# tkoolen/Parametron.jl

Hardware: AMD Instinct MI355X
Metric: QP re-evaluations/sec (Q,q,C,d rebuild) at n=4096 (higher is better)
Workload: dtype f64; 1 GPU; C2 dense least-squares QP: n=4096 vars, A 4096x4096, m=512 equality rows, fp64; canonical Q,q,const + C,d MOI triplets; n=4096, r=4096, m=512, objective_mode=canonical, instances_per_gpu=1, parallelism=single GPU, replay=tape

## Files before the change

parametron.jl_amd/csrc/gram.hip:

```cpp
#include <algorithm>
#include <memory>
#include <vector>

#include "streams.h"

#ifndef PMT_GRAM_ABL_NO_LINEAR
#define PMT_GRAM_ABL_NO_LINEAR 0
#endif

namespace pmt {

constexpr size_t PAIR_FLAG_BYTES = 4096;
constexpr int DELIVER_ORDER_W = 1;

__global__ __launch_bounds__(256) void gram_linear_kernel(const double *__restrict__ A, int64_t lda, int64_t rows, int64_t cols,
                                                          const int64_t *__restrict__ xvar, const double *__restrict__ b, int sign,
                                                          int moi, const int64_t *__restrict__ varmap, LT *__restrict__ out_lin) {
    const int64_t col = (int64_t)blockIdx.x * 4 + (threadIdx.x >> 6);
    if (col >= cols) return;
    const int lane = threadIdx.x & 63;
    const double *a = A + col * lda;
    double acc = 0.0;
    if (b && sign)
        for (int64_t i = lane; i < rows; i += 64) acc += signed_const(b[i], sign) * a[i];
// ... 218 lines not shown
static int release_group(const DeliverPlan &d, SideStream *side, int grp, hipStream_t s) {
    const dma::Signal flag{0, reinterpret_cast<int64_t *>(static_cast<char *>(side->counters) + FLAGS_OFFSET) + grp};
    return dma::launch_signal_store(d.sig->engine ? d.sig->dep[grp] : flag, s);
}

static int deliver_submit(const DeliverPlan &d, SideStream *side) {
    if (!d.sig->engine) {
        char *cb = static_cast<char *>(side->counters);
        if (int rc = launch_courier(d.src, d.host_dev, reinterpret_cast<long long *>(cb + FLAGS_OFFSET), reinterpret_cast<unsigned *>(cb + DONE_OFFSET),
                                    side->err_dev, d.ngroups, d.gbeg, d.gend, side->fetch)) return rc;
        PMT_HIP_CHECK(hipEventRecord(side->fetch_done, side->fetch));
        side->fetch_pending = true;
        return PMT_OK;
    }
    auto submit = [p = d]() -> int {
        for (int i = 0; i < p.ngroups; ++i)
            if (int rc = dma::copy_to_host(p.sig->eng, p.host + p.gbeg[i], p.src + p.gbeg[i], sizeof(double) * (size_t)(p.gend[i] - p.gbeg[i]),
                                           &p.sig->dep[i], p.sig->done, 1)) return rc;
        return PMT_OK;
    };
    d.sig->pending = true;
    side->dma_pending.emplace_back(d.sig->eng, d.sig->done);
    side->keepalive.push_back(d.sig);
    if (!side->in_replay) return submit();
    side->deferred.push_back(submit);
    return PMT_OK;
}

static int fork_side(SideStream *side, hipStream_t s) {
    PMT_HIP_CHECK(hipEventRecord(side->fork, s));
    PMT_HIP_CHECK(hipStreamWaitEvent(side->stream, side->fork, 0));
    return PMT_OK;
}

static int fused_node(const GramArgs &g, SideStream *side, hipStream_t s) {
    int rc = launch_gram_tall(g.A, g.lda, g.rows, g.cols, g.xvar, g.b, g.sign, g.moi, g.varmap, g.out_quad, g.out_csc, g.alpha, g.out_lin,
                              g.out_const, g.workspace, s);
    if (!rc && side && side->in_replay) rc = fork_side(side, s);
    const int64_t nt = cdiv(g.cols, ST);
    if (!rc && nt > 1)
        rc = launch_gram_sk(g.A, g.lda, g.rows, g.cols, g.xvar, g.varmap, g.moi, g.out_quad, g.out_csc, g.alpha, g.workspace, 0, 0, nt * (nt - 1) / 2,
                            nullptr, 0, nullptr, s, 1);
    return rc;
}

static int mid_node(const GramArgs &g, SideStream *side, hipStream_t s) {
    PMT_REQUIRE(side && side->counters && (size_t)gram_mid_counters(g.cols) * sizeof(unsigned) <= MID_COUNTER_BYTES, PMT_STATE_ERROR,
                "quad_gram: no auxiliary state for this stream");
    int rc = launch_gram_mid(g.A, g.lda, g.rows, g.cols, g.xvar, g.b, g.sign, g.moi, g.varmap, g.out_quad, g.out_csc, g.alpha, g.out_lin,
                             g.out_const, g.workspace, reinterpret_cast<unsigned *>(static_cast<char *>(side->counters) + MID_OFFSET), s);
    return !rc && side->in_replay ? fork_side(side, s) : rc;
}

static int stream_k_node(const GramArgs &g, bool staged, const DeliverPlan &d, SideStream *side, hipStream_t s) {
    hipStream_t s2 = side ? side->stream : s;
    if (side) { if (int rc = fork_side(side, s)) return rc; }
    const int64_t rows = g.rows, cols = g.cols;
    int rc = PMT_OK;
    double *scratch = g.workspace ? reinterpret_cast<double *>(static_cast<char *>(g.workspace) + gram_sk_workspace_bytes(rows, cols)) : nullptr;
    const int nsplit = (scratch && g.b && g.sign) ? linear_splits(rows, cols) : 1;
    if (PMT_GRAM_ABL_NO_LINEAR) {
    } else if (cols > 0 && nsplit > 1) {
        const int64_t chunk = 64 * cdiv(cdiv(rows, nsplit), 64);
        PMT_LAUNCH(gram_linear_split_kernel, dim3((unsigned)cdiv(cols, 4), (unsigned)nsplit), dim3(256), 0, s2, g.A, g.lda, rows, cols, g.b, g.sign, chunk, scratch);
        PMT_LAUNCH(gram_linear_finish_kernel, dim3((unsigned)cdiv(cols, 256)), dim3(256), 0, s2, scratch, nsplit, cols, g.xvar, g.moi, g.varmap, g.out_lin);
        rc = check_launch("gram_linear_split_kernel");
    } else if (cols > 0) {
        PMT_LAUNCH(gram_linear_kernel, dim3((unsigned)cdiv(cols, 4)), dim3(256), 0, s2, g.A, g.lda, rows, cols, g.xvar, g.b, g.sign, g.moi, g.varmap, g.out_lin);
        rc = check_launch("gram_linear_kernel");
    }
    double *chains = scratch ? scratch + (size_t)linear_splits(rows, cols) * (size_t)cols : nullptr;
    const int order = constant_order(staged ? GramForm::StreamKStaged : GramForm::StreamK, rows, cols).order;
    auto const_part = [=]() -> int {
        int rc2 = PMT_OK;
        if (order == 5) rc2 = launch_gram_mid_constant(g.b, g.sign, rows, g.out_const, s2);
        else if (g.b && g.sign && rows > 0) rc2 = launch_blocked_dot(g.b, g.sign, g.b, g.sign, rows, chains, g.out_const, s2, order);
        else if (hipMemsetAsync(g.out_const, 0, sizeof(double), s2) != hipSuccess) rc2 = fail(PMT_HIP_ERROR, "hipMemsetAsync(out_const)");
        if (side) { PMT_HIP_CHECK(hipEventRecord(side->join2, side->stream)); PMT_HIP_CHECK(hipStreamWaitEvent(s, side->join2, 0)); }
        return rc2;
    };
    const bool defer_const = side && side->in_replay;
    if (!rc && defer_const) side->deferred.push_back(const_part);
    if (side) PMT_HIP_CHECK(hipEventRecord(side->join, side->stream));
    if (!rc && cols > 0 && !staged) rc = launch_gram_sk(g.A, g.lda, rows, cols, g.xvar, g.varmap, g.moi, g.out_quad, g.out_csc, g.alpha, g.workspace, 0, 0, -1,
                                                        nullptr, 0, nullptr, s);
    else if (!rc && cols > 0) {
        unsigned *pair_flags = g.workspace ? reinterpret_cast<unsigned *>(static_cast<char *>(g.workspace) + gram_sk_workspace_bytes(rows, cols) - PAIR_FLAG_BYTES) : nullptr;
        if (pair_flags) PMT_HIP_CHECK(hipMemsetAsync(pair_flags, 0, PAIR_FLAG_BYTES, s));
        for (int st = 0; !rc && st < d.nstages; ++st) {
// ... 103 lines not shown
```

parametron.jl_amd/csrc/gram_mid.hip:

```cpp
#include "gram_common.h"

#ifndef PMT_MID_WPS
#define PMT_MID_WPS 1
#endif
#ifndef PMT_MID_G
#define PMT_MID_G 256
#endif
#ifndef PMT_MID_MAXWG
#define PMT_MID_MAXWG 2304
#endif
#ifndef PMT_MID_D
#define PMT_MID_D 2
#endif
#ifndef PMT_MID_GROUP_US
#define PMT_MID_GROUP_US 1.15
#endif
#ifndef PMT_MID_TAIL_US
#define PMT_MID_TAIL_US 0.95
#endif
#ifndef PMT_MID_SB
#define PMT_MID_SB 8
#endif
#ifndef PMT_MID_FB
#define PMT_MID_FB 4
#endif
#ifndef PMT_MID_FORMAL
#if defined(__HIP_DEVICE_COMPILE__) && !defined(__gfx950__) && !defined(__gfx942__)
#define PMT_MID_FORMAL 1
#else
#define PMT_MID_FORMAL 0
#endif
#endif

#ifdef PMT_MID_TRACE
__device__ unsigned long long g_mid_trace[1024 * 8];
#define MID_STAMP(k) do { if (threadIdx.x == 0 && blockIdx.x < 1024) g_mid_trace[blockIdx.x * 8 + (k)] = wall_clock64(); } while (0)
extern "C" int pmt_mid_trace_read(unsigned long long *host) {
    return hipMemcpyFromSymbol(host, HIP_SYMBOL(g_mid_trace), sizeof(unsigned long long) * 1024 * 8) == hipSuccess ? 0 : 1;
}
#else
#define MID_STAMP(k) do { } while (0)
#endif

namespace pmt {

constexpr int MT = 64;
constexpr int MACC = 64;
constexpr int MPART = MACC * 64;
constexpr int MSTRIDE = MPART + MT + 8;
constexpr int MPITCH = MT + 1;
constexpr int MFG = 8;
constexpr int MCNT = 16;
constexpr int MQBUF = 4 * 2048;
constexpr int MFLAG = MQBUF + 4 * MT;
constexpr int MMAPS = MFLAG + 8;
constexpr int MSH = MMAPS + 2 * MT;

struct MidArgs {
    const double *A; int64_t lda, rows, cols;
    const double *b; int sign;
    const int64_t *xvar; const int64_t *varmap; int moi;
    QT *out_quad; double *out_csc; double alpha; LT *out_lin; double *out_const;
    int nb;
    int n_off, s_off, s_diag;
    int gpc_off, gpc_diag;
    int n_tail, s_tail, gpc_tail;
    double *ws;
    unsigned *counters;
    int xcd;
    int persist, total;
    unsigned *tickets;
};

struct MidPlan { int nb, n_off, s_off, s_diag, gpc_off, gpc_diag, n_tail, s_tail, gpc_tail, wgs; };
// ... 128 lines not shown
        for (int tm = 0; tm < (DIAG ? c + 1 : 4); ++tm) {
            const int a = (tm * 4 + c) * 4;
            acc[a] = __builtin_amdgcn_mfma_f64_4x4x4f64(buf[tm].y, bv[c][0].y, acc[a], 0, 0, 0);
        }
    __builtin_amdgcn_sched_barrier(0);
#pragma unroll
    for (int c = 0; c < NC; ++c) {
#pragma unroll
        for (int r = 1; r < 4; ++r)
#pragma unroll
            for (int tm = 0; tm < (DIAG ? c + 1 : 4); ++tm) {
                const int a = (tm * 4 + c) * 4 + r;
                acc[a] = __builtin_amdgcn_mfma_f64_4x4x4f64(buf[tm].x, bv[c][r].x, acc[a], 0, 0, 0);
            }
#pragma unroll
        for (int r = 1; r < 4; ++r)
#pragma unroll
            for (int tm = 0; tm < (DIAG ? c + 1 : 4); ++tm) {
                const int a = (tm * 4 + c) * 4 + r;
                acc[a] = __builtin_amdgcn_mfma_f64_4x4x4f64(buf[tm].y, bv[c][r].y, acc[a], 0, 0, 0);
            }
    }
    if (DIAG) {
        const double c0 = signed_const(cb.x, sign), c1 = signed_const(cb.y, sign);
#pragma unroll
        for (int t = 0; t < 4; ++t) qacc[t] = __builtin_amdgcn_mfma_f64_4x4x4f64(buf[t].x, c0, qacc[t], 0, 0, 0);
#pragma unroll
        for (int t = 0; t < 4; ++t) qacc[t] = __builtin_amdgcn_mfma_f64_4x4x4f64(buf[t].y, c1, qacc[t], 0, 0, 0);
    }
}

#define MID_SB() __builtin_amdgcn_sched_barrier(0)
template <bool DIAG>
__device__ __forceinline__ void mid_step(const MidArgs &g, double *__restrict__ rot, int64_t next_row0, unsigned (&voff)[DIAG ? 4 : 8],
                                         f64x2 (&buf)[DIAG ? 4 : 8], f64x2 &cb, int sign, int lane, double (&acc)[MACC], double (&qacc)[4]) {
    constexpr int BO = DIAG ? 0 : 4;
    const int lm = lane & 15, lrow = lane & 48, lk = lane >> 4;
    const char *base = reinterpret_cast<const char *>(g.A + next_row0);
    auto reload = [&](int t) {
        asm volatile("" : "+v"(voff[t]));
        buf[t] = *reinterpret_cast<const f64x2 *>(base + voff[t]);
    };
    f64x2 bv[4][4];
#pragma unroll
    for (int c = 0; c < 4; ++c) bv[c][0] = buf[BO + c];
    auto lds_op = [&](int i) {
        if (i < 4) *reinterpret_cast<f64x2 *>(rot + (i * 64 + lane) * 2) = buf[BO + i];
        else {
            const int c = (i - 4) / 3, r = 1 + (i - 4) % 3;
            bv[c][r] = *reinterpret_cast<const f64x2 *>(rot + (c * 64 + lrow + ((lm + 4 * r) & 15)) * 2);
        }
    };
    MID_SB();
    int k = 0;
#pragma unroll
    for (int pass = 0; pass < 2; ++pass)
#pragma unroll
        for (int c = 0; c < 4; ++c)
#pragma unroll
            for (int tm = 0; tm < (DIAG ? c + 1 : 4); ++tm) {
                const int a = (tm * 4 + c) * 4;
                acc[a] = __builtin_amdgcn_mfma_f64_4x4x4f64(pass ? buf[tm].y : buf[tm].x, pass ? bv[c][0].y : bv[c][0].x, acc[a], 0, 0, 0);
                if (k < 16) { MID_SB(); lds_op(k); MID_SB(); }
                ++k;
            }
    if (DIAG) {
        const double c0 = signed_const(cb.x, sign), c1 = signed_const(cb.y, sign);
#pragma unroll
        for (int t = 0; t < 4; ++t) qacc[t] = __builtin_amdgcn_mfma_f64_4x4x4f64(buf[t].x, c0, qacc[t], 0, 0, 0);
#pragma unroll
        for (int t = 0; t < 4; ++t) qacc[t] = __builtin_amdgcn_mfma_f64_4x4x4f64(buf[t].y, c1, qacc[t], 0, 0, 0);
        MID_SB();
        cb = *reinterpret_cast<const f64x2 *>((g.b ? g.b : g.A) + next_row0 + 2 * lk);
    }
// ... 182 lines not shown
#endif
}

template <bool DIAG>
__device__ __forceinline__ void mid_fold(const double *p, int count, int64_t stride, int tid, double (&sum)[16], double &qs) {
#pragma unroll
    for (int u = 0; u < 16; ++u) sum[u] = 0.0;
    qs = 0.0;
    for (int c0 = 0; c0 < count; c0 += PMT_MID_FB) {
        double v[PMT_MID_FB][16], qv[PMT_MID_FB];
#pragma unroll
        for (int cc = 0; cc < PMT_MID_FB; ++cc) {
            const double *pc = p + (int64_t)min(c0 + cc, count - 1) * stride;
#pragma unroll
            for (int u = 0; u < 16; ++u) {
                const int a = (tid >> 6) + 4 * u;
                v[cc][u] = 0.0;
                if (mid_used(DIAG, a)) v[cc][u] = mid_get(pc + tid + 256 * u);
            }
            qv[cc] = 0.0;
            if (DIAG && tid < MT) qv[cc] = mid_get(pc + MPART + tid);
        }
#pragma unroll
        for (int cc = 0; cc < PMT_MID_FB; ++cc) {
            const bool live = c0 + cc < count;
#pragma unroll
            for (int u = 0; u < 16; ++u) { const double t = sum[u] + v[cc][u]; sum[u] = live ? t : sum[u]; }
            const double t = qs + qv[cc];
            qs = live ? t : qs;
        }
    }
}

template <bool DIAG, bool FAST>
__device__ __forceinline__ void mid_body(const MidArgs &g, double *sh, int tid, int jb, int kb, int chunk, int nchunk, int gpc, int first_wg, unsigned *counter) {
    constexpr int NG = DIAG ? 4 : 8;
    constexpr int D = PMT_MID_D;
    const int lane = tid & 63;
    const int wave = __builtin_amdgcn_readfirstlane(tid >> 6);
    const int lm = lane & 15, lk = lane >> 4;
    const int64_t cj0 = (int64_t)jb * MT, ck0 = (int64_t)kb * MT;
    const int ngroups = (int)((g.rows + 7) >> 3);
    const int g0 = chunk * gpc + wave, g1 = min((chunk + 1) * gpc, ngroups);
    const int my = g1 > g0 ? (g1 - g0 + 3) / 4 : 0;
    const bool ragged = FAST && (g.rows & 7) && my > 0 && g0 + 4 * (my - 1) == ngroups - 1;
    const int nfast = ragged ? my - 1 : my;

    MID_STAMP(0);
    mid_maps(g, sh, tid, jb, kb);
    double acc[MACC], qacc[4] = {0.0, 0.0, 0.0, 0.0};
#pragma unroll
    for (int a = 0; a < MACC; ++a) acc[a] = 0.0;
    unsigned voff[NG];
#pragma unroll
    for (int t = 0; t < NG; ++t) voff[t] = (unsigned)((min((t < 4 ? cj0 : ck0) + 16 * (t & 3) + lm, g.cols - 1) * g.lda + 2 * lk) * 8);
    double *rot = sh + wave * 512;
    f64x2 buf[D][NG], cb[D];
    auto row_of = [&](int s) { return (int64_t)(g0 + 4 * min(s, max(nfast - 1, 0))) * 8; };
    if (nfast > 0) {
#pragma unroll
        for (int d = 0; d < D; ++d) mid_load<DIAG, FAST>(g, row_of(d), lane, cj0, ck0, voff, buf[d], cb[d]);
        if (FAST) {
            int s0 = 0;
            for (; s0 + D <= nfast; s0 += D) {
#pragma unroll
                for (int d = 0; d < D; ++d) mid_step<DIAG>(g, rot, row_of(s0 + d + D), voff, buf[d], cb[d], g.sign, lane, acc, qacc);
            }
#pragma unroll
            for (int d = 0; d < D - 1; ++d)
                if (s0 + d < nfast) mid_compute<DIAG>(rot, buf[d], cb[d], g.sign, lane, acc, qacc);
        } else {
            for (int s0 = 0; s0 < nfast; s0 += D) {
#pragma unroll
                for (int d = 0; d < D; ++d) {
                    if (s0 + d < nfast) mid_compute<DIAG>(rot, buf[d], cb[d], g.sign, lane, acc, qacc);
                    mid_load<DIAG, FAST>(g, row_of(s0 + d + D), lane, cj0, ck0, voff, buf[d], cb[d]);
                }
            }
        }
    }
    if (ragged) {
        mid_load<DIAG, false>(g, (int64_t)(ngroups - 1) * 8, lane, cj0, ck0, voff, buf[0], cb[0]);
        mid_compute<DIAG>(rot, buf[0], cb[0], g.sign, lane, acc, qacc);
    }

    MID_STAMP(1);
    unsigned *flag = reinterpret_cast<unsigned *>(sh + MFLAG);
    double *w = g.ws + (int64_t)(first_wg + chunk) * MSTRIDE;
    __syncthreads();
    if (wave == 0) mid_tail<DIAG, 0>(g, sh, lane, acc, qacc, nchunk, w);
    else if (wave == 1) mid_tail<DIAG, 1>(g, sh, lane, acc, qacc, nchunk, w);
    else if (wave == 2) mid_tail<DIAG, 2>(g, sh, lane, acc, qacc, nchunk, w);
    else mid_tail<DIAG, 3>(g, sh, lane, acc, qacc, nchunk, w);
    MID_STAMP(2);
    if (nchunk > 1) {
        const bool two = nchunk > MFG;
        const int gfirst = two ? (chunk / MFG) * MFG : 0;
        const int n1 = two ? min(MFG, nchunk - gfirst) : nchunk;
        unsigned *c1 = two ? counter + 1 + chunk / MFG : counter;
        __syncthreads();
        if (tid == 0) *flag = __hip_atomic_fetch_add(c1, 1u, __ATOMIC_RELAXED, __HIP_MEMORY_SCOPE_AGENT);
        __syncthreads();
        MID_STAMP(3);
        if (*flag != (unsigned)(n1 - 1)) return;
#if PMT_MID_FORMAL
        __builtin_amdgcn_fence(__ATOMIC_ACQUIRE, "agent");
#endif
        if (tid == 0) __hip_atomic_store(c1, 0u, __ATOMIC_RELAXED, __HIP_MEMORY_SCOPE_AGENT);
        double sum[16], qs;
        double *p = g.ws + (int64_t)(first_wg + gfirst) * MSTRIDE;
        mid_fold<DIAG>(p, n1, MSTRIDE, tid, sum, qs);
        if (two) {
#pragma unroll
            for (int u = 0; u < 16; ++u) if (mid_used(DIAG, (tid >> 6) + 4 * u)) mid_put(p + tid + 256 * u, sum[u]);
            if (DIAG && tid < MT) mid_put(p + MPART + tid, qs);
#if PMT_MID_FORMAL
            __builtin_amdgcn_fence(__ATOMIC_RELEASE, "agent");
#else
            __builtin_amdgcn_s_waitcnt(0);
#endif
            __syncthreads();
            if (tid == 0) *flag = __hip_atomic_fetch_add(counter, 1u, __ATOMIC_RELAXED, __HIP_MEMORY_SCOPE_AGENT);
            __syncthreads();
            const int ng = (nchunk + MFG - 1) / MFG;
            if (*flag != (unsigned)(ng - 1)) return;
#if PMT_MID_FORMAL
            __builtin_amdgcn_fence(__ATOMIC_ACQUIRE, "agent");
#endif
            if (tid == 0) __hip_atomic_store(counter, 0u, __ATOMIC_RELAXED, __HIP_MEMORY_SCOPE_AGENT);
            mid_fold<DIAG>(g.ws + (int64_t)first_wg * MSTRIDE, ng, (int64_t)MFG * MSTRIDE, tid, sum, qs);
        }
        __syncthreads();
        MID_STAMP(4);
#pragma unroll
        for (int u = 0; u < 16; ++u) {
            const int a = (tid >> 6) + 4 * u;
            if (!mid_used(DIAG, a)) continue;
            int row, col;
            mid_pos(lane, a, row, col);
            sh[row * MPITCH + col] = sum[u];
        }
        if (DIAG && tid < MT) sh[MT * MPITCH + tid] = qs;
    }
    __syncthreads();
    MID_STAMP(5);
    mid_epilogue(g, sh, tid, jb, kb);
#ifdef PMT_MID_TRACE
    __builtin_amdgcn_s_waitcnt(0);
    MID_STAMP(6);
#endif
}

__device__ __forceinline__ int mid_xcd_rank(int id, int base, int n) {
    const int x = id & 7, end = base + n;
    int start = 0;
    for (int y = 0; y < x; ++y) {
        const int fy = base + ((y - base) & 7);
        start += fy < end ? ((end - 1 - fy) >> 3) + 1 : 0;
    }
    return start + ((id - (base + ((x - base) & 7))) >> 3);
}

__device__ __forceinline__ void mid_tile_of(int t, int nb, int &jb, int &kb) {
    constexpr int SB = PMT_MID_SB;
    const int nsb = (nb + SB - 1) / SB;
    for (int K = 0; K < nsb; ++K) {
        const int wK = min(SB, nb - SB * K);
        for (int J = 0; J <= K; ++J) {
            const int cnt = J < K ? SB * wK : wK * (wK - 1) / 2;
            if (t >= cnt) { t -= cnt; continue; }
            if (J < K) { jb = SB * J + t / wK; kb = SB * K + t % wK; return; }
            int kk = 1;
            while (t >= kk) { t -= kk; ++kk; }
            jb = SB * K + t; kb = SB * K + kk;
            return;
        }
    }
    jb = 0; kb = 1;
}

template <bool FAST>
__device__ __forceinline__ void mid_item(const MidArgs &g, double *sh, int tid, int id) {
    const int nbody = g.n_off - g.n_tail, wbody = nbody * g.s_off, noff = wbody + g.n_tail * g.s_tail;
    if (id < noff) {
        const bool tail = id >= wbody;
        const int base = tail ? wbody : 0, ntile = tail ? g.n_tail : nbody, nch = tail ? g.s_tail : g.s_off;
        const int k = g.xcd ? mid_xcd_rank(id, base, ntile * nch) : ((id - base) % nch) * ntile + (id - base) / nch;
        const int chunk = k / ntile;
        const int rank = (tail ? nbody : 0) + (k - chunk * ntile);
        int t = rank, jb, kb;
        if (g.xcd) mid_tile_of(t, g.nb, jb, kb);
        else {
            kb = 1;
            while (t >= kb) { t -= kb; ++kb; }
            jb = t;
        }
        const int first = tail ? wbody + (rank - nbody) * g.s_tail : rank * g.s_off;
        mid_body<false, FAST>(g, sh, tid, jb, kb, chunk, nch, tail ? g.gpc_tail : g.gpc_off, first, g.counters + rank * MCNT);
        return;
    }
    if (id < noff + g.nb * g.s_diag) {
        const int k = g.xcd ? mid_xcd_rank(id, noff, g.nb * g.s_diag) : ((id - noff) % g.s_diag) * g.nb + (id - noff) / g.s_diag;
        const int chunk = k / g.nb, jb = k - chunk * g.nb;
        mid_body<true, FAST>(g, sh, tid, jb, jb, chunk, g.s_diag, g.gpc_diag, noff + jb * g.s_diag, g.counters + (g.n_off + jb) * MCNT);
        return;
    }
    mid_constant(g, sh, tid);
}

template <bool FAST>
__global__ __launch_bounds__(256, PMT_MID_WPS) void gram_mid_kernel(MidArgs g) {
    __shared__ double sh[MSH];
    __shared__ int next_id;
    const int tid = threadIdx.x;
    const int x = blockIdx.x & 7, per = gridDim.x >> 3;
    int id = blockIdx.x;
    for (;;) {
        mid_item<FAST>(g, sh, tid, id);
        if (!g.persist) return;
        __syncthreads();
        if (tid == 0) next_id = x + 8 * (per + (int)__hip_atomic_fetch_add(g.tickets + x, 1u, __ATOMIC_RELAXED, __HIP_MEMORY_SCOPE_AGENT));
        __syncthreads();
        id = next_id;
        if (id >= g.total) break;
    }
    if (tid == 0) {
        const unsigned gone = __hip_atomic_fetch_add(g.tickets + 8, 1u, __ATOMIC_RELAXED, __HIP_MEMORY_SCOPE_AGENT);
        if (gone == gridDim.x - 1) {
#pragma unroll
            for (int i = 0; i < 9; ++i) __hip_atomic_store(g.tickets + i, 0u, __ATOMIC_RELAXED, __HIP_MEMORY_SCOPE_AGENT);
        }
    }
}

__global__ __launch_bounds__(256) void gram_mid_constant_kernel(MidArgs g) {
    __shared__ double sh[8];
    mid_constant(g, sh, threadIdx.x);
}
int launch_gram_mid_constant(const double *b, int sign, int64_t rows, double *out_const, hipStream_t s) {
    MidArgs g = {};
    g.rows = rows; g.b = (b && sign) ? b : nullptr; g.sign = g.b ? sign : 0; g.out_const = out_const;
    PMT_LAUNCH_NAMED("gram_mid_constant_kernel", gram_mid_constant_kernel, dim3(1), dim3(256), 0, s, g);
    return check_launch("gram_mid_constant_kernel");
}

size_t gram_mid_workspace_bytes(int64_t rows, int64_t cols) {
    if (cols <= 0) return 0;
    const MidPlan p = mid_plan(rows, cols);
    return sizeof(double) * (size_t)p.wgs * MSTRIDE;
}
int gram_mid_counters(int64_t cols) { const int nb = (int)cdiv(cols, MT); return MCNT * (nb * (nb + 1) / 2) + 16; }

int launch_gram_mid(const double *A, int64_t lda, int64_t rows, int64_t cols, const int64_t *xvar, const double *b, int sign, int moi,
                    const int64_t *varmap, pmt_quadratic_term *out_quad, double *out_csc, double alpha, pmt_linear_term *out_lin,
                    double *out_const, void *workspace, unsigned *counters, hipStream_t s) {
    if (!workspace || !counters) return fail(PMT_INVALID_ARGUMENT, "quad_gram: workspace required");
    const MidPlan p = mid_plan(rows, cols);
    MidArgs g;
// ... 20 lines not shown
```

parametron.jl_amd/csrc/plan.hip:

```cpp
#include <algorithm>
#include <atomic>
#include <cstring>
#include <mutex>
#include <unordered_map>
#include <vector>

#include <memory>

#include "streams.h"

namespace pmt {

static thread_local std::string g_last_error;
void set_error(const std::string &msg) { g_last_error = msg; }
int fail(int code, const std::string &msg) { g_last_error = msg; return code; }

}

struct pmt_plan {
    int device = 0;
    hipStream_t stream = nullptr;
    bool owns_stream = false;
    bool recording = false;
    std::vector<void *> allocations;
// ... 642 lines not shown
extern "C" int pmt_plan_end_record(pmt_plan *plan) {
    PMT_REQUIRE(plan, PMT_INVALID_ARGUMENT, "plan_end_record: null plan");
    PMT_REQUIRE(plan->recording, PMT_STATE_ERROR, "plan is not recording");
    plan->recording = false;
    plan->record_lane = 0;
    return build_exec(plan);
}

extern "C" int pmt_plan_set_fusion(pmt_plan *plan, int on) {
    PMT_REQUIRE(plan, PMT_INVALID_ARGUMENT, "plan_set_fusion: null plan");
    PMT_REQUIRE(!plan->recording, PMT_STATE_ERROR, "plan_set_fusion: the plan is recording");
    PMT_REQUIRE(!plan->graph_exec, PMT_STATE_ERROR, "plan_set_fusion: the plan's graph is already instantiated");
    plan->fusion = on != 0;
    PMT_HIP_CHECK(hipSetDevice(plan->device));
    PMT_HIP_CHECK(hipStreamSynchronize(plan->stream));
    return build_exec(plan);
}

extern "C" int pmt_plan_fused_phases(const pmt_plan *plan) { return plan ? plan->fused_phases : 0; }
extern "C" int pmt_plan_fused_workgroups(const pmt_plan *plan) { return plan ? plan->fused_workgroups : 0; }

extern "C" int pmt_plan_fused(const pmt_plan *plan, int *groups, int *nodes, int64_t *exec_length) {
    PMT_REQUIRE(plan, PMT_INVALID_ARGUMENT, "plan_fused: null plan");
    if (groups) *groups = plan->fused_groups;
    if (nodes) *nodes = plan->fused_nodes;
    if (exec_length) *exec_length = (int64_t)plan->exec.size();
    return PMT_OK;
}


static int replay(pmt_plan *plan, hipStream_t s) {
    if (!plan->fetch_events.empty())
        if (int rc = pmt::fetch_fence(s)) return rc;
    pmt::replay_begin(s);
    struct End { hipStream_t s; int rc = PMT_OK; bool done = false; int finish() { if (!done) { done = true; rc = pmt::replay_end(s); } return rc; } ~End() { finish(); } } end{s};
    hipStream_t side = nullptr;
    bool any = false;
    for (char l : plan->exec_lanes) any |= (l != 0);
    if (any && (side = pmt::side_stream_of(s))) {
        if (!plan->lane_fork) {
            PMT_HIP_CHECK(hipEventCreateWithFlags(&plan->lane_fork, hipEventDisableTiming));
            PMT_HIP_CHECK(hipEventCreateWithFlags(&plan->lane_join, hipEventDisableTiming));
        }
        PMT_HIP_CHECK(hipEventRecord(plan->lane_fork, s));
    }
    bool forked = false;
    bool side_used = false;
    for (size_t i = 0; side && i < plan->exec.size(); ++i)
        if (plan->exec_lanes[i] == 3) {
            side_used = true;
            if (int rc = plan->exec[i](side)) return rc;
        }
    for (size_t i = 0; side && i < plan->exec.size(); ++i) {
        if (plan->exec_lanes[i] != 2) continue;
        if (!forked) { PMT_HIP_CHECK(hipStreamWaitEvent(side, plan->lane_fork, 0)); forked = true; }
        if (int rc = plan->exec[i](side)) return rc;
    }
    for (size_t i = 0; i < plan->exec.size(); ++i) {
        hipStream_t target = s;
        if (side && plan->exec_lanes[i] >= 2) continue;
        if (side && plan->exec_lanes[i]) {
            if (!forked) { PMT_HIP_CHECK(hipStreamWaitEvent(side, plan->lane_fork, 0)); forked = true; }
            target = side;
        }
        int rc = plan->exec[i](target);
        if (rc) return rc;
    }
    if (forked || side_used) {
        PMT_HIP_CHECK(hipEventRecord(plan->lane_join, side));
        PMT_HIP_CHECK(hipStreamWaitEvent(s, plan->lane_join, 0));
    }
// ... 98 lines not shown
```

parametron.jl_amd/csrc/streams.h:

```cpp
#pragma once
#include <memory>
#include <vector>

#include "dma.h"
#include "gram_common.h"

namespace pmt {

struct SideStream {
    hipStream_t stream = nullptr; hipEvent_t fork = nullptr, join = nullptr, join2 = nullptr; int device = -1;
    void *counters = nullptr;
    int *err_host = nullptr, *err_dev = nullptr;
    hipStream_t fetch = nullptr; hipEvent_t fetch_done = nullptr; bool fetch_pending = false;
    std::vector<std::pair<dma::Engine *, dma::Signal>> dma_pending;
    std::vector<std::shared_ptr<void>> keepalive;
    bool in_replay = false;
    std::vector<std::function<int()>> deferred;
};
constexpr int ERR_COURIER = 1, ERR_PAIR_FOLD = 2;
constexpr size_t PROGRESS_OFFSET = 0;
constexpr size_t FLAGS_OFFSET = PROGRESS_OFFSET + MAXGROUPS * sizeof(unsigned long long);
constexpr size_t DONE_OFFSET = FLAGS_OFFSET + MAXGROUPS * sizeof(long long);
constexpr size_t MID_OFFSET = DONE_OFFSET + 2 * sizeof(unsigned);
constexpr size_t MID_COUNTER_BYTES = 135168;
constexpr size_t COUNTER_BYTES = MID_OFFSET + MID_COUNTER_BYTES;

SideStream *side_stream(hipStream_t s);
int ensure_fetch_stream(SideStream *ss);
int wait_dma_pending(SideStream *ss);
inline hipStream_t side_stream_of(hipStream_t s) { SideStream *ss = side_stream(s); return ss ? ss->stream : nullptr; }
void retain_side_stream(hipStream_t s);
void release_side_stream(hipStream_t s);
int fetch_async(hipStream_t s, hipStream_t after, hipEvent_t order_event, void *host_dst, const void *device_src, size_t bytes, FetchState *st, FetchRect r);
int fetch_fence(hipStream_t s);
int fetch_synchronize(hipStream_t s);
void replay_begin(hipStream_t s);
int replay_end(hipStream_t s);
int gram_after_deferred(hipStream_t s, std::function<int()> f);

void *host_device_pointer(void *host);
int launch_courier(const double *src, double *dst_dev, long long *ready, unsigned *done, int *error, int ngroups, const int64_t *gbeg, const int64_t *gend, hipStream_t s);
int launch_to_host(const void *src, void *dst_dev, size_t bytes, hipStream_t s);
int launch_to_host_2d(const void *src, size_t src_pitch, void *dst_dev, size_t dst_pitch, size_t width_bytes, size_t height, hipStream_t s);

}
```

parametron.jl_amd/csrc/streams.hip:

```cpp
#include <cstring>
#include <mutex>
#include <unordered_map>

#include "streams.h"

namespace pmt {

static std::mutex g_side_mu;
static std::unordered_map<hipStream_t, SideStream> g_side;
static const long long ARMED[MAXGROUPS] = {1, 1, 1, 1, 1, 1, 1, 1, 1, 1, 1, 1, 1, 1, 1, 1};

static void destroy_side(SideStream &ss) {
    for (hipStream_t st : {ss.stream, ss.fetch}) if (st) { (void)hipStreamSynchronize(st); (void)hipStreamDestroy(st); }
    for (hipEvent_t e : {ss.fork, ss.join, ss.join2, ss.fetch_done}) if (e) (void)hipEventDestroy(e);
    (void)wait_dma_pending(&ss);
    if (ss.counters) (void)hipFree(ss.counters);
    if (ss.err_host) (void)hipHostFree(ss.err_host);
}

SideStream *side_stream(hipStream_t s) {
#ifdef PMT_TUNING
    static const bool enabled = [] { const char *e = getenv("PMT_GRAM_SIDE_STREAM"); return !(e && e[0] == '0'); }();
    if (!enabled) return nullptr;
#endif
// ... 124 lines not shown
static void trace_dma_pending(SideStream *ss, hipStream_t s) {
    std::vector<long> last(ss->dma_pending.size(), -100);
    bool stream_done = false;
    const double t0 = host_us();
    for (;;) {
        bool all = true;
        for (size_t i = 0; i < ss->dma_pending.size(); ++i) {
            const long v = (long)*ss->dma_pending[i].second.value;
            if (v != last[i]) { fprintf(stderr, "[trace +%.0f us] transfer set %zu: %ld left\n", host_us() - g_replay_t0, i, v); last[i] = v; }
            if (v > 0) all = false;
        }
        if (!stream_done && hipStreamQuery(s) == hipSuccess) { stream_done = true; fprintf(stderr, "[trace +%.0f us] the plan's stream is idle\n", host_us() - g_replay_t0); }
        if ((all && stream_done) || host_us() - t0 > 1e6) break;
    }
}
#endif

int wait_dma_pending(SideStream *ss) {
    int rc = PMT_OK;
    for (auto &p : ss->dma_pending) { const int r = dma::wait(p.first, p.second, 10.0); if (r && !rc) rc = r; }
    ss->dma_pending.clear();
    ss->keepalive.clear();
    return rc;
}

int fetch_fence(hipStream_t s) {
    SideStream *ss = find_side(s);
    if (!ss) return PMT_OK;
    if (int rc = wait_dma_pending(ss)) return rc;
    if (ss->fetch_pending) { PMT_HIP_CHECK(hipStreamWaitEvent(s, ss->fetch_done, 0)); ss->fetch_pending = false; }
    return PMT_OK;
}

void replay_begin(hipStream_t s) {
#ifdef PMT_TUNING
    g_replay_t0 = host_us();
#endif
    if (SideStream *ss = find_side(s)) ss->in_replay = true;
}
int replay_end(hipStream_t s) {
    SideStream *ss = find_side(s);
    if (!ss) return PMT_OK;
    ss->in_replay = false;
    int rc = PMT_OK;
    for (auto &f : ss->deferred) { const int r = f(); if (r && !rc) rc = r; }
    ss->deferred.clear();
    return rc;
}

int gram_after_deferred(hipStream_t s, std::function<int()> f) {
    SideStream *ss = find_side(s);
    if (!ss || !ss->in_replay || ss->deferred.empty()) return f();
    ss->deferred.push_back(std::move(f));
    return PMT_OK;
}

int fetch_synchronize(hipStream_t s) {
    SideStream *ss = find_side(s);
    if (!ss) return PMT_OK;
#ifdef PMT_TUNING
    { const char *e = getenv("PMT_DMA_DEBUG"); if (e && e[0] == '2') trace_dma_pending(ss, s); }
#endif
    int rc = wait_dma_pending(ss);
    if (!rc && ss->fetch) PMT_HIP_CHECK(hipStreamSynchronize(ss->fetch));
    const int err = ss->err_host ? __atomic_exchange_n(ss->err_host, 0, __ATOMIC_ACQ_REL) : 0;
    if (err == ERR_COURIER) {
        PMT_HIP_CHECK(hipMemset(ss->counters, 0, COUNTER_BYTES));
        PMT_HIP_CHECK(hipMemcpy(static_cast<char *>(ss->counters) + FLAGS_OFFSET, ARMED, sizeof ARMED, hipMemcpyHostToDevice));
        return fail(PMT_HIP_ERROR, "host delivery: the courier saw no progress of the contraction for 2 s and gave up; the host arrays are incomplete");
    }
    if (err == ERR_PAIR_FOLD)
        return fail(PMT_HIP_ERROR, "host delivery: a split tile of the contraction never received its first half (pair fold); the tile was "
                                   "written as NaN and the delivered quadratic coefficients are invalid");
    if (err) return fail(PMT_HIP_ERROR, "host delivery: unknown device error " + std::to_string(err));
    return rc;
}
// ... 8 lines not shown
```

Measured before the change: 894.8 re-evaluations/s.

## Prefetch next work item's tiles in persistent mid Gram kernel and skip needless forks

In the persistent mid-size Gram kernel, each workgroup now draws its next ticket early, decodes the next off-diagonal tile, and uses the last step of the current fast loop to prefetch the next tile's first rows into registers. This hides the global-load latency between work items. The cost is more register pressure from a persistent 8-wide prefetch buffer plus added control complexity. Separately, the side-stream fork event is now recorded during replay only when some lane actually runs on the side stream, which drops an event record and wait per replay. Trace instrumentation is extended but is compiled only under a debug macro.

```diff
diff --git a/parametron.jl_amd/csrc/gram.hip b/parametron.jl_amd/csrc/gram.hip
--- a/parametron.jl_amd/csrc/gram.hip
+++ b/parametron.jl_amd/csrc/gram.hip
@@ -274,11 +274,12 @@
     PMT_HIP_CHECK(hipStreamWaitEvent(side->stream, side->fork, 0));
     return PMT_OK;
 }
+static bool forks_in_replay(const SideStream *side) { return side && side->in_replay && side->side_work; }
 
 static int fused_node(const GramArgs &g, SideStream *side, hipStream_t s) {
     int rc = launch_gram_tall(g.A, g.lda, g.rows, g.cols, g.xvar, g.b, g.sign, g.moi, g.varmap, g.out_quad, g.out_csc, g.alpha, g.out_lin,
                               g.out_const, g.workspace, s);
-    if (!rc && side && side->in_replay) rc = fork_side(side, s);
+    if (!rc && forks_in_replay(side)) rc = fork_side(side, s);
     const int64_t nt = cdiv(g.cols, ST);
     if (!rc && nt > 1)
         rc = launch_gram_sk(g.A, g.lda, g.rows, g.cols, g.xvar, g.varmap, g.moi, g.out_quad, g.out_csc, g.alpha, g.workspace, 0, 0, nt * (nt - 1) / 2,
@@ -291,12 +292,13 @@
                 "quad_gram: no auxiliary state for this stream");
     int rc = launch_gram_mid(g.A, g.lda, g.rows, g.cols, g.xvar, g.b, g.sign, g.moi, g.varmap, g.out_quad, g.out_csc, g.alpha, g.out_lin,
                              g.out_const, g.workspace, reinterpret_cast<unsigned *>(static_cast<char *>(side->counters) + MID_OFFSET), s);
-    return !rc && side->in_replay ? fork_side(side, s) : rc;
+    return !rc && forks_in_replay(side) ? fork_side(side, s) : rc;
 }
 
 static int stream_k_node(const GramArgs &g, bool staged, const DeliverPlan &d, SideStream *side, hipStream_t s) {
     hipStream_t s2 = side ? side->stream : s;
     if (side) { if (int rc = fork_side(side, s)) return rc; }
+    if (side && side->in_replay) side->side_work = true;
     const int64_t rows = g.rows, cols = g.cols;
     int rc = PMT_OK;
     double *scratch = g.workspace ? reinterpret_cast<double *>(static_cast<char *>(g.workspace) + gram_sk_workspace_bytes(rows, cols)) : nullptr;
diff --git a/parametron.jl_amd/csrc/gram_mid.hip b/parametron.jl_amd/csrc/gram_mid.hip
--- a/parametron.jl_amd/csrc/gram_mid.hip
+++ b/parametron.jl_amd/csrc/gram_mid.hip
@@ -34,12 +34,27 @@
 
 #ifdef PMT_MID_TRACE
 __device__ unsigned long long g_mid_trace[1024 * 8];
-#define MID_STAMP(k) do { if (threadIdx.x == 0 && blockIdx.x < 1024) g_mid_trace[blockIdx.x * 8 + (k)] = wall_clock64(); } while (0)
+__device__ unsigned long long g_mid_walk[1024 * 8];
+#define MID_TRACE_WORDS 8
+__device__ __forceinline__ void mid_walk_note(unsigned long long *w, int k, unsigned long long t) {
+    if (k == 0) { if (w[0]) w[4] += t - w[7]; else w[5] = t; w[0] += 1; }
+    else if (k == 1) w[1] += t - w[7];
+    else if (k == 3 || k == 5) { w[2] += t - w[7]; w[6] = t; }
+    else if (k == 6) { w[3] += t - w[7]; w[6] = t; }
+    else return;
+    w[7] = t;
+}
+#define MID_STAMP(k) do { if (threadIdx.x == 0 && blockIdx.x < 1024) { const unsigned long long t_ = wall_clock64(); g_mid_trace[blockIdx.x * 8 + (k)] = t_; \
+                          mid_walk_note(reinterpret_cast<unsigned long long *>(sh + MSH), (k), t_); } } while (0)
 extern "C" int pmt_mid_trace_read(unsigned long long *host) {
     return hipMemcpyFromSymbol(host, HIP_SYMBOL(g_mid_trace), sizeof(unsigned long long) * 1024 * 8) == hipSuccess ? 0 : 1;
 }
+extern "C" int pmt_mid_walk_read(unsigned long long *host) {
+    return hipMemcpyFromSymbol(host, HIP_SYMBOL(g_mid_walk), sizeof(unsigned long long) * 1024 * 8) == hipSuccess ? 0 : 1;
+}
 #else
 #define MID_STAMP(k) do { } while (0)
+#define MID_TRACE_WORDS 0
 #endif
 
 namespace pmt {
@@ -234,14 +249,14 @@
 
 #define MID_SB() __builtin_amdgcn_sched_barrier(0)
 template <bool DIAG>
-__device__ __forceinline__ void mid_step(const MidArgs &g, double *__restrict__ rot, int64_t next_row0, unsigned (&voff)[DIAG ? 4 : 8],
-                                         f64x2 (&buf)[DIAG ? 4 : 8], f64x2 &cb, int sign, int lane, double (&acc)[MACC], double (&qacc)[4]) {
+__device__ __forceinline__ void mid_step(const MidArgs &g, double *__restrict__ rot, int64_t next_row0, const char *base_a, const char *base_b,
+                                         unsigned (&voff)[DIAG ? 4 : 8], f64x2 (&buf)[DIAG ? 4 : 8], f64x2 &cb, int sign, int lane,
+                                         double (&acc)[MACC], double (&qacc)[4]) {
     constexpr int BO = DIAG ? 0 : 4;
     const int lm = lane & 15, lrow = lane & 48, lk = lane >> 4;
-    const char *base = reinterpret_cast<const char *>(g.A + next_row0);
     auto reload = [&](int t) {
         asm volatile("" : "+v"(voff[t]));
-        buf[t] = *reinterpret_cast<const f64x2 *>(base + voff[t]);
+        buf[t] = *reinterpret_cast<const f64x2 *>((t < 4 ? base_a : base_b) + voff[t]);
     };
     f64x2 bv[4][4];
 #pragma unroll
@@ -490,10 +505,34 @@
     }
 }
 
+struct MidWalk {
+    bool early;
+    unsigned *ticket; int id0;
+    int *slot;
+    int drawn;
+    bool next_full; int njb, nkb, nrank;
+    bool pre;
+};
+
+template <int N>
+__device__ __forceinline__ void mid_forget(f64x2 (&buf)[PMT_MID_D][N]) {
+#pragma unroll
+    for (int d = 0; d < PMT_MID_D; ++d)
+#pragma unroll
+        for (int t = 0; t < N; ++t) asm volatile("" : "=v"(buf[d][t].x), "=v"(buf[d][t].y));
+}
+
+template <bool DIAG>
+__device__ __forceinline__ auto &mid_buf(f64x2 (&own)[PMT_MID_D][4], f64x2 (&walk)[PMT_MID_D][8]) {
+    if constexpr (DIAG) return own; else return walk;
+}
+
 template <bool DIAG, bool FAST>
-__device__ __forceinline__ void mid_body(const MidArgs &g, double *sh, int tid, int jb, int kb, int chunk, int nchunk, int gpc, int first_wg, unsigned *counter) {
+__device__ __forceinline__ void mid_body(const MidArgs &g, double *sh, int tid, int jb, int kb, int chunk, int nchunk, int gpc, int first_wg, unsigned *counter,
+                                         MidWalk &wk, f64x2 (&pbuf)[PMT_MID_D][8]) {
     constexpr int NG = DIAG ? 4 : 8;
     constexpr int D = PMT_MID_D;
+    asm volatile("" : "+v"(tid));
     const int lane = tid & 63;
     const int wave = __builtin_amdgcn_readfirstlane(tid >> 6);
     const int lm = lane & 15, lk = lane >> 4;
@@ -513,16 +552,33 @@
 #pragma unroll
     for (int t = 0; t < NG; ++t) voff[t] = (unsigned)((min((t < 4 ? cj0 : ck0) + 16 * (t & 3) + lm, g.cols - 1) * g.lda + 2 * lk) * 8);
     double *rot = sh + wave * 512;
-    f64x2 buf[D][NG], cb[D];
+    f64x2 dbuf[D][4], cb[D];
+    auto &buf = mid_buf<DIAG>(dbuf, pbuf);
     auto row_of = [&](int s) { return (int64_t)(g0 + 4 * min(s, max(nfast - 1, 0))) * 8; };
+    const bool pre = !DIAG && wk.pre;
+    bool pf = false;
+    if (!DIAG && FAST) pf = wk.early && wk.next_full && nchunk == 1 && !ragged && nfast > 0 && nfast % D == 0 && (int64_t)(kb + 1) * MT <= g.cols;
+    const int ahead_at = __builtin_amdgcn_readfirstlane(pf ? nfast - D : -1);
+    const int64_t shift_a = pf ? ((int64_t)wk.njb * MT - cj0) * g.lda * 8 : 0, shift_b = pf ? ((int64_t)wk.nkb * MT - ck0) * g.lda * 8 : 0;
     if (nfast > 0) {
-#pragma unroll
-        for (int d = 0; d < D; ++d) mid_load<DIAG, FAST>(g, row_of(d), lane, cj0, ck0, voff, buf[d], cb[d]);
+        if (!pre) {
+#pragma unroll
+            for (int d = 0; d < D; ++d) {
+                __builtin_amdgcn_sched_barrier(0);
+                mid_load<DIAG, FAST>(g, row_of(d), lane, cj0, ck0, voff, buf[d], cb[d]);
+            }
+            __builtin_amdgcn_sched_barrier(0);
+        }
         if (FAST) {
             int s0 = 0;
             for (; s0 + D <= nfast; s0 += D) {
-#pragma unroll
-                for (int d = 0; d < D; ++d) mid_step<DIAG>(g, rot, row_of(s0 + d + D), voff, buf[d], cb[d], g.sign, lane, acc, qacc);
+                const bool ahead = s0 == ahead_at;
+#pragma unroll
+                for (int d = 0; d < D; ++d) {
+                    const int64_t row = ahead ? row_of(d) : row_of(s0 + d + D);
+                    const char *base = reinterpret_cast<const char *>(g.A + row);
+                    mid_step<DIAG>(g, rot, row, base + (ahead ? shift_a : 0), base + (ahead ? shift_b : 0), voff, buf[d], cb[d], g.sign, lane, acc, qacc);
+                }
             }
 #pragma unroll
             for (int d = 0; d < D - 1; ++d)
@@ -543,6 +599,9 @@
     }
 
     MID_STAMP(1);
+    wk.pre = pf;
+    unsigned drawn = 0;
+    if (!DIAG && wk.early && tid == 0) drawn = __hip_atomic_fetch_add(wk.ticket, 1u, __ATOMIC_RELAXED, __HIP_MEMORY_SCOPE_AGENT);
     unsigned *flag = reinterpret_cast<unsigned *>(sh + MFLAG);
     double *w = g.ws + (int64_t)(first_wg + chunk) * MSTRIDE;
     __syncthreads();
@@ -560,7 +619,7 @@
         if (tid == 0) *flag = __hip_atomic_fetch_add(c1, 1u, __ATOMIC_RELAXED, __HIP_MEMORY_SCOPE_AGENT);
         __syncthreads();
         MID_STAMP(3);
-        if (*flag != (unsigned)(n1 - 1)) return;
+        if (*flag != (unsigned)(n1 - 1)) { mid_forget(buf); return; }
 #if PMT_MID_FORMAL
         __builtin_amdgcn_fence(__ATOMIC_ACQUIRE, "agent");
 #endif
@@ -581,7 +640,7 @@
             if (tid == 0) *flag = __hip_atomic_fetch_add(counter, 1u, __ATOMIC_RELAXED, __HIP_MEMORY_SCOPE_AGENT);
             __syncthreads();
             const int ng = (nchunk + MFG - 1) / MFG;
-            if (*flag != (unsigned)(ng - 1)) return;
+            if (*flag != (unsigned)(ng - 1)) { mid_forget(buf); return; }
 #if PMT_MID_FORMAL
             __builtin_amdgcn_fence(__ATOMIC_ACQUIRE, "agent");
 #endif
@@ -599,8 +658,11 @@
             sh[row * MPITCH + col] = sum[u];
         }
         if (DIAG && tid < MT) sh[MT * MPITCH + tid] = qs;
-    }
+        mid_forget(buf);
+    }
+    if (!DIAG && wk.early && tid == 0) *wk.slot = wk.id0 + 8 * (int)drawn;
     __syncthreads();
+    if (!DIAG && wk.early) wk.drawn = *wk.slot;
     MID_STAMP(5);
     mid_epilogue(g, sh, tid, jb, kb);
 #ifdef PMT_MID_TRACE
@@ -637,8 +699,9 @@
     jb = 0; kb = 1;
 }
 
-template <bool FAST>
-__device__ __forceinline__ void mid_item(const MidArgs &g, double *sh, int tid, int id) {
+struct MidItem { int kind, jb, kb, chunk, nch, gpc, first, rank; };
+__device__ __forceinline__ MidItem mid_decode(const MidArgs &g, int id) {
+    MidItem it = {2, 0, 0, 0, 1, 0, 0, 0};
     const int nbody = g.n_off - g.n_tail, wbody = nbody * g.s_off, noff = wbody + g.n_tail * g.s_tail;
     if (id < noff) {
         const bool tail = id >= wbody;
@@ -653,35 +716,83 @@
             while (t >= kb) { t -= kb; ++kb; }
             jb = t;
         }
-        const int first = tail ? wbody + (rank - nbody) * g.s_tail : rank * g.s_off;
-        mid_body<false, FAST>(g, sh, tid, jb, kb, chunk, nch, tail ? g.gpc_tail : g.gpc_off, first, g.counters + rank * MCNT);
-        return;
+        it.kind = 0; it.jb = jb; it.kb = kb; it.chunk = chunk; it.nch = nch; it.gpc = tail ? g.gpc_tail : g.gpc_off;
+        it.first = tail ? wbody + (rank - nbody) * g.s_tail : rank * g.s_off;
+        it.rank = rank;
+        return it;
     }
     if (id < noff + g.nb * g.s_diag) {
         const int k = g.xcd ? mid_xcd_rank(id, noff, g.nb * g.s_diag) : ((id - noff) % g.s_diag) * g.nb + (id - noff) / g.s_diag;
         const int chunk = k / g.nb, jb = k - chunk * g.nb;
-        mid_body<true, FAST>(g, sh, tid, jb, jb, chunk, g.s_diag, g.gpc_diag, noff + jb * g.s_diag, g.counters + (g.n_off + jb) * MCNT);
+        it.kind = 1; it.jb = jb; it.kb = jb; it.chunk = chunk; it.nch = g.s_diag; it.gpc = g.gpc_diag; it.first = noff + jb * g.s_diag; it.rank = g.n_off + jb;
+    }
+    return it;
+}
+
+template <bool FAST>
+__device__ __forceinline__ void mid_item(const MidArgs &g, double *sh, int tid, const MidItem &it, MidWalk &wk, f64x2 (&pbuf)[PMT_MID_D][8]) {
+    if (it.kind == 0) {
+        mid_body<false, FAST>(g, sh, tid, it.jb, it.kb, it.chunk, it.nch, it.gpc, it.first, g.counters + it.rank * MCNT, wk, pbuf);
         return;
     }
-    mid_constant(g, sh, tid);
+    wk.pre = false;
+    if (it.kind == 1) mid_body<true, FAST>(g, sh, tid, it.jb, it.kb, it.chunk, it.nch, it.gpc, it.first, g.counters + it.rank * MCNT, wk, pbuf);
+    else mid_constant(g, sh, tid);
+    mid_forget(pbuf);
 }
 
 template <bool FAST>
 __global__ __launch_bounds__(256, PMT_MID_WPS) void gram_mid_kernel(MidArgs g) {
-    __shared__ double sh[MSH];
-    __shared__ int next_id;
+    __shared__ double sh[MSH + MID_TRACE_WORDS];
+    __shared__ int next_id, ahead_id;
     const int tid = threadIdx.x;
     const int x = blockIdx.x & 7, per = gridDim.x >> 3;
-    int id = blockIdx.x;
+#ifdef PMT_MID_TRACE
+    if (tid == 0) for (int i = 0; i < MID_TRACE_WORDS; ++i) reinterpret_cast<unsigned long long *>(sh + MSH)[i] = 0;
+#endif
+    f64x2 pbuf[PMT_MID_D][8];
+    MidWalk wk = {};
+    wk.ticket = g.tickets + x; wk.id0 = x + 8 * per; wk.slot = &ahead_id;
+    const int wbody = (g.n_off - g.n_tail) * g.s_off;
+    const bool look = FAST && g.persist && g.s_off == 1;
+    int id = blockIdx.x, hand = -1;
+    if (look) {
+        if (tid == 0) next_id = wk.id0 + 8 * (int)__hip_atomic_fetch_add(wk.ticket, 1u, __ATOMIC_RELAXED, __HIP_MEMORY_SCOPE_AGENT);
+        __syncthreads();
+        hand = next_id;
+    }
+    MidItem cur = mid_decode(g, id);
     for (;;) {
-        mid_item<FAST>(g, sh, tid, id);
+        wk.early = hand >= 0 && hand < wbody;
+        wk.next_full = false;
+        if (wk.early) {
+            const MidItem nx = mid_decode(g, hand);
+            wk.next_full = (int64_t)(nx.kb + 1) * MT <= g.cols;
+            wk.njb = nx.jb; wk.nkb = nx.kb; wk.nrank = nx.rank;
+        }
+        mid_item<FAST>(g, sh, tid, cur, wk, pbuf);
         if (!g.persist) return;
         __syncthreads();
-        if (tid == 0) next_id = x + 8 * (per + (int)__hip_atomic_fetch_add(g.tickets + x, 1u, __ATOMIC_RELAXED, __HIP_MEMORY_SCOPE_AGENT));
-        __syncthreads();
-        id = next_id;
+        if (wk.early) {
+            id = hand; hand = wk.drawn;
+            cur.jb = wk.njb; cur.kb = wk.nkb; cur.first = cur.rank = wk.nrank;
+            continue;
+        }
+        if (hand >= 0) { id = hand; hand = -1; }
+        else {
+            if (tid == 0) next_id = wk.id0 + 8 * (int)__hip_atomic_fetch_add(wk.ticket, 1u, __ATOMIC_RELAXED, __HIP_MEMORY_SCOPE_AGENT);
+            __syncthreads();
+            id = next_id;
+        }
         if (id >= g.total) break;
-    }
+        cur = mid_decode(g, id);
+    }
+#ifdef PMT_MID_TRACE
+    if (tid == 0 && blockIdx.x < 1024) {
+        for (int i = 0; i < 7; ++i) g_mid_walk[blockIdx.x * 8 + i] = reinterpret_cast<unsigned long long *>(sh + MSH)[i];
+        g_mid_walk[blockIdx.x * 8 + 7] = wall_clock64();
+    }
+#endif
     if (tid == 0) {
         const unsigned gone = __hip_atomic_fetch_add(g.tickets + 8, 1u, __ATOMIC_RELAXED, __HIP_MEMORY_SCOPE_AGENT);
         if (gone == gridDim.x - 1) {
diff --git a/parametron.jl_amd/csrc/plan.hip b/parametron.jl_amd/csrc/plan.hip
--- a/parametron.jl_amd/csrc/plan.hip
+++ b/parametron.jl_amd/csrc/plan.hip
@@ -698,11 +698,11 @@
 static int replay(pmt_plan *plan, hipStream_t s) {
     if (!plan->fetch_events.empty())
         if (int rc = pmt::fetch_fence(s)) return rc;
-    pmt::replay_begin(s);
+    bool any = false;
+    for (char l : plan->exec_lanes) any |= (l != 0);
+    pmt::replay_begin(s, any);
     struct End { hipStream_t s; int rc = PMT_OK; bool done = false; int finish() { if (!done) { done = true; rc = pmt::replay_end(s); } return rc; } ~End() { finish(); } } end{s};
     hipStream_t side = nullptr;
-    bool any = false;
-    for (char l : plan->exec_lanes) any |= (l != 0);
     if (any && (side = pmt::side_stream_of(s))) {
         if (!plan->lane_fork) {
             PMT_HIP_CHECK(hipEventCreateWithFlags(&plan->lane_fork, hipEventDisableTiming));
diff --git a/parametron.jl_amd/csrc/streams.h b/parametron.jl_amd/csrc/streams.h
--- a/parametron.jl_amd/csrc/streams.h
+++ b/parametron.jl_amd/csrc/streams.h
@@ -15,6 +15,7 @@
     std::vector<std::pair<dma::Engine *, dma::Signal>> dma_pending;
     std::vector<std::shared_ptr<void>> keepalive;
     bool in_replay = false;
+    bool side_work = false;
     std::vector<std::function<int()>> deferred;
 };
 constexpr int ERR_COURIER = 1, ERR_PAIR_FOLD = 2;
@@ -34,7 +35,7 @@
 int fetch_async(hipStream_t s, hipStream_t after, hipEvent_t order_event, void *host_dst, const void *device_src, size_t bytes, FetchState *st, FetchRect r);
 int fetch_fence(hipStream_t s);
 int fetch_synchronize(hipStream_t s);
-void replay_begin(hipStream_t s);
+void replay_begin(hipStream_t s, bool side_work);
 int replay_end(hipStream_t s);
 int gram_after_deferred(hipStream_t s, std::function<int()> f);
 
diff --git a/parametron.jl_amd/csrc/streams.hip b/parametron.jl_amd/csrc/streams.hip
--- a/parametron.jl_amd/csrc/streams.hip
+++ b/parametron.jl_amd/csrc/streams.hip
@@ -180,16 +180,17 @@
     return PMT_OK;
 }
 
-void replay_begin(hipStream_t s) {
+void replay_begin(hipStream_t s, bool side_work) {
 #ifdef PMT_TUNING
     g_replay_t0 = host_us();
 #endif
-    if (SideStream *ss = find_side(s)) ss->in_replay = true;
+    if (SideStream *ss = find_side(s)) { ss->in_replay = true; ss->side_work = side_work; }
 }
 int replay_end(hipStream_t s) {
     SideStream *ss = find_side(s);
     if (!ss) return PMT_OK;
     ss->in_replay = false;
+    ss->side_work = false;
     int rc = PMT_OK;
     for (auto &f : ss->deferred) { const int r = f(); if (r && !rc) rc = r; }
     ss->deferred.clear();
```

New measurement: 919.5 re-evaluations/s (median of 6 runs). +2.8%, better.
